# ViliamVadocz/tak

Measured on AMD Instinct MI355X. Metric: MCTS node-expansions/sec (5x5 Tak, 400 sims/move, 4096 games/GPU), higher is better.
Workload: dtype f32

## Files before the change

### tak_amd/csrc/conv_mainloop.cuh

```cuda
#pragma once
#include <hip/hip_runtime.h>
#include <stdint.h>

#include <utility>

namespace tg {

using f32x16 = __attribute__((ext_vector_type(16))) float;
using f32x4 = __attribute__((ext_vector_type(4))) float;
constexpr int LDS_PAD = 4;
constexpr int LDS_PAD16 = 8;


template <int RTW>
__device__ __forceinline__ void conv_tap_masks(int rows, int n, int nsq, int rho0, int (&vmask)[RTW]) {
#pragma unroll
    for (int j = 0; j < RTW; j++) {
        int rho = rho0 + j * 16;
        int p = rho / nsq;
        int sq = rho - p * nsq;
        int y = sq / n, x = sq - y * n;
        int m = 0;
#pragma unroll
        for (int t = 0; t < 9; t++) {
// ... 138 lines not shown
#pragma unroll
                for (int j = 0; j < H1; j++) { TG_HALO_MFMA(j, t, s) }
            __builtin_amdgcn_sched_barrier(0);
            if (SPLIT && s % CH == 0 && s > 0) {
#pragma unroll
                for (int j = H1; j < RTW; j++) { acc[j] += part[j]; asm volatile("" : "+v"(acc[j])); }
            }
            f32x4 w2;
            if (s < ROW - 2) {
                w2 = TG_HALO_W(wchunk);
            } else {
                const bool on = dy == 2;
                const __amdgpu_buffer_rsrc_t r = __builtin_amdgcn_make_buffer_rsrc((void*)(on ? wnext : wlayer), 0, (int)(9 * CH * WCHUNK), 0x00020000);
                w2 = __builtin_bit_cast(f32x4, __builtin_amdgcn_raw_buffer_load_b128(r, wlane, (int)((on ? s - (ROW - 2) : wchunk) * WCHUNK), 0));
            }
            wchunk++;
            if (s + 1 < ROW) {
#pragma unroll
                for (int j = 0; j < H1; j++) a[j] = lds4[ad[j] + TG_HALO_OFF2(s + 1)];
            } else {
#pragma unroll
                for (int j = H1; j < RTW; j++) ad[j] += RS * P4;
                if (dy < 2) {
#pragma unroll
                    for (int j = 0; j < H1; j++) { ad[j] += RS * P4; a[j] = lds4[ad[j] + TG_HALO_OFF2(0)]; }
                }
            }
            __builtin_amdgcn_sched_barrier(0);
#pragma unroll
            for (int t = 0; t < 4; t++)
#pragma unroll
                for (int j = H1; j < RTW; j++) { TG_HALO_MFMA(j, t, s) }
            __builtin_amdgcn_sched_barrier(0);
            if (SPLIT && s % CH == CH - 1) {
#pragma unroll
                for (int j = 0; j < (s == ROW - 1 ? RTW : H1); j++) { acc[j] += part[j]; asm volatile("" : "+v"(acc[j])); }
            }
            w0 = w1;
            w1 = w2;
        }
    }
#undef TG_HALO_MFMA
#undef TG_HALO_OFF2
#ifndef TG_NO_PRIO_TURNS
    __builtin_amdgcn_s_setprio(0);
#endif
#undef TG_HALO_OFF
#undef TG_HALO_W
}

constexpr int SQ_NB = 5;
template <int CH> constexpr int sq_image_cell4() { return 4 * CH + 2; }
template <int CH> constexpr int sq_image_pitch4() {
    constexpr int c = SQ_NB * SQ_NB * sq_image_cell4<CH>();
    return c + ((2 - c) % 16 + 16) % 16;
}
static_assert(sq_image_pitch4<4>() == 450, "C2: 16 positions = 115 200 B");
__host__ __device__ constexpr int sq_tiles(int rg) { return rg == 0 ? 13 : 12; }
__host__ __device__ constexpr int sq_tile(int rg, int j) { return rg == 0 ? (j < 12 ? j : 14) : (j < 2 ? 12 + j : 13 + j); }
__host__ __device__ constexpr bool sq_tap_on(int sq, int tap) {
    const int y = sq / SQ_NB + tap / 3 - 1, x = sq % SQ_NB + tap % 3 - 1;
    return y >= 0 && y < SQ_NB && x >= 0 && x < SQ_NB;
}
__host__ __device__ constexpr int sq_tap_count(int rg, int tap) {
    int c = 0;
    for (int j = 0; j < sq_tiles(rg); j++) c += sq_tap_on(sq_tile(rg, j), tap) ? 1 : 0;
    return c;
}
__host__ __device__ constexpr int sq_tap_tile(int rg, int tap, int k) {
    for (int j = 0; j < sq_tiles(rg); j++)
        if (sq_tap_on(sq_tile(rg, j), tap) && k-- == 0) return j;
    return -1;
}
static_assert(sq_tap_count(0, 0) + sq_tap_count(0, 1) + sq_tap_count(0, 2) + sq_tap_count(0, 3) + sq_tap_count(0, 4) + sq_tap_count(0, 5) +
                      sq_tap_count(0, 6) + sq_tap_count(0, 7) + sq_tap_count(0, 8) == 86, "row group 0: 86 on-board taps");
static_assert(sq_tap_count(1, 0) + sq_tap_count(1, 1) + sq_tap_count(1, 2) + sq_tap_count(1, 3) + sq_tap_count(1, 4) + sq_tap_count(1, 5) +
                      sq_tap_count(1, 6) + sq_tap_count(1, 7) + sq_tap_count(1, 8) == 83, "row group 1: 83 on-board taps");

template <typename Fn, int... I>
__device__ __forceinline__ void static_for_impl(Fn& f, std::integer_sequence<int, I...>) { (f(std::integral_constant<int, I>{}), ...); }
template <int N, typename Fn>
__device__ __forceinline__ void static_for(Fn&& f) { static_for_impl(f, std::make_integer_sequence<int, N>{}); }

template <int RG, int CH>
__device__ __forceinline__ void conv_mainloop_sq(const f32x4* __restrict__ img4, const float* __restrict__ wlayer,
                                                 const float* __restrict__ wnext, uint32_t wlane, f32x4 (&acc)[13], const int turn,
                                                 f32x4& w0, f32x4& w1) {
    constexpr int STEPS = 9 * CH, ROW = 3 * CH, CP4 = sq_image_cell4<CH>();
    constexpr size_t WCHUNK = (size_t)16 * CH * 4 * 16;
    static_assert(sq_tiles(RG) <= 13, "acc holds 13 tiles");
#ifndef TG_PRIO_PERIOD
#define TG_PRIO_PERIOD 2
#endif
    const __amdgpu_buffer_rsrc_t wrsrc = __builtin_amdgcn_make_buffer_rsrc((void*)wlayer, 0, (int)(9 * CH * WCHUNK), 0x00020000);
    const __amdgpu_buffer_rsrc_t nrsrc = __builtin_amdgcn_make_buffer_rsrc((void*)wnext, 0, (int)(9 * CH * WCHUNK), 0x00020000);
    constexpr auto cnt = [](int s) { return sq_tap_count(RG, s / CH); };
    constexpr auto h1 = [](int s) { return (sq_tap_count(RG, s / CH) + 1) / 2; };
    constexpr auto off = [](int s, int k) {
        return (sq_tile(RG, sq_tap_tile(RG, s / CH, k)) + (s / CH / 3 - 1) * SQ_NB + (s / CH % 3 - 1)) * CP4 + (s % CH) * 4;
    };
    f32x4 a1[7], a2[7];
    static_for<7>([&](auto K) {
        constexpr int k = decltype(K)::value;
        if constexpr (k < h1(0)) a1[k] = img4[off(0, k)];
    });
    static_for<STEPS>([&](auto S) {
        constexpr int s = decltype(S)::value;
#ifndef TG_NO_PRIO_TURNS
        if constexpr (s % TG_PRIO_PERIOD == 0) {
            if ((((s % ROW) / TG_PRIO_PERIOD + s / ROW) & 1) == turn) __builtin_amdgcn_s_setprio(1);
            else __builtin_amdgcn_s_setprio(0);
        }
#endif
        static_for<7>([&](auto K) {
            constexpr int k = decltype(K)::value;
            if constexpr (h1(s) + k < cnt(s)) a2[k] = img4[off(s, h1(s) + k)];
        });
        __builtin_amdgcn_sched_barrier(0);
        static_for<4>([&](auto T) {
            static_for<7>([&](auto K) {
                constexpr int t = decltype(T)::value, k = decltype(K)::value;
                if constexpr (k < h1(s)) {
                    constexpr int j = sq_tap_tile(RG, s / CH, k);
                    acc[j] = __builtin_amdgcn_mfma_f32_16x16x4f32(w0[t], a1[k][t], acc[j], 0, 0, 0);
                }
            });
        });
        __builtin_amdgcn_sched_barrier(0);
        f32x4 w2;
        if constexpr (s < STEPS - 2) w2 = __builtin_bit_cast(f32x4, __builtin_amdgcn_raw_buffer_load_b128(wrsrc, wlane, (int)((s + 2) * WCHUNK), 0));
        else w2 = __builtin_bit_cast(f32x4, __builtin_amdgcn_raw_buffer_load_b128(nrsrc, wlane, (int)((s - (STEPS - 2)) * WCHUNK), 0));
        if constexpr (s + 1 < STEPS) {
            static_for<7>([&](auto K) {
                constexpr int k = decltype(K)::value;
                if constexpr (k < h1(s + 1)) a1[k] = img4[off(s + 1, k)];
            });
        }
        __builtin_amdgcn_sched_barrier(0);
        static_for<4>([&](auto T) {
            static_for<7>([&](auto K) {
                constexpr int t = decltype(T)::value, k = decltype(K)::value;
                if constexpr (h1(s) + k < cnt(s)) {
                    constexpr int j = sq_tap_tile(RG, s / CH, h1(s) + k);
                    acc[j] = __builtin_amdgcn_mfma_f32_16x16x4f32(w0[t], a2[k][t], acc[j], 0, 0, 0);
                }
            });
        });
        __builtin_amdgcn_sched_barrier(0);
        w0 = w1;
        w1 = w2;
    });
#ifndef TG_NO_PRIO_TURNS
    __builtin_amdgcn_s_setprio(0);
#endif
}

template <int CH, int COT = CH>
__device__ __forceinline__ void conv_halo_first_weights(const float* __restrict__ wlayer, uint32_t wlane, f32x4& w0, f32x4& w1) {
    constexpr size_t WCHUNK = (size_t)16 * COT * 4 * 16;
    const __amdgpu_buffer_rsrc_t wrsrc = __builtin_amdgcn_make_buffer_rsrc((void*)wlayer, 0, (int)(9 * CH * WCHUNK), 0x00020000);
    w0 = __builtin_bit_cast(f32x4, __builtin_amdgcn_raw_buffer_load_b128(wrsrc, wlane, 0, 0));
    w1 = __builtin_bit_cast(f32x4, __builtin_amdgcn_raw_buffer_load_b128(wrsrc, wlane, (int)WCHUNK, 0));
}

}
```

### tak_amd/csrc/net.hip

```cpp
#include <cmath>
#include <cstdlib>
#include <cstring>

#include "engine.h"
#include "kernels.h"
#include "softmax.cuh"
#include "rng.cuh"

namespace tg {

struct ConvLayer {
    DevBuf w, b;
    int cin_pad = 0;
    int cout = 0, cout_pad = 0;
};

struct Net {
    std::map<std::string, std::vector<float>> tensors;
    bool ready = false;
    int F = 0, R = 0, cin = 0, cin_pad = 0;
    ConvLayer conv0;
    std::vector<ConvLayer> res1, res2;
    ConvLayer policy_conv;
    DevBuf policy_w, policy_b;
// ... 460 lines not shown
    TG_HIP(n->y.ensure(mb * nsq * F * 4));
    size_t logit_row = e->cfg.policy_head == TG_HEAD_CONV ? (size_t)nsq * n->policy_conv.cout_pad : (size_t)std::max(n->policy_np, n->s3_np);
    TG_HIP(n->logits.ensure(mb * logit_row * 4));
    TG_HIP(n->planes_nhwc.ensure(mb * nsq * n->cin_pad * 4));
    const bool s3fc = n->s3 && n->s3_fc_on;
    n->fc_stats_on = e->cfg.policy_head == TG_HEAD_FC5 && n->value_in_fc && !env_on("TG_NO_FC_STATS") && e->policy_size + 1 <= FC_TILES * 16 &&
                     (s3fc ? n->s3_np >= FC_TILES * 16 : fc_stats_supported(nsq * F, n->policy_np, n->policy_np));
    n->fc_stat_blocks = n->fc_stats_on ? FC_STAT_BLOCKS : 0;
    n->fc_stat_stride = n->fc_stats_on ? FC_STAT_STRIDE : 0;
    if (n->fc_stats_on) TG_HIP(n->fc_stats.ensure(mb * (size_t)n->fc_stat_stride * 2 * 4));
    n->ready = true;
    return TG_OK;
}

static int net_forward_impl(TgEngine* e, int nb, const float* d_planes, const uint8_t* d_states, float* d_policy, float* d_eval);

int net_forward_dev(TgEngine* e, int nb, const float* d_planes, float* d_policy, float* d_eval) {
    return net_forward_impl(e, nb, d_planes, nullptr, d_policy, d_eval);
}

bool net_takes_states(const TgEngine* e) { return net_ready(e) && (e->net->fused || e->net->s3); }

const float* net_fc_logits(const TgEngine* e, int* ld) {
    if (!net_ready(e)) return nullptr;
    const Net* n = e->net;
    if (e->cfg.policy_head != TG_HEAD_FC5 || !n->value_in_fc || e->policy_size > 2048) return nullptr;
    if (n->s3 && !n->s3_fc_on) return nullptr;
    *ld = n->s3 && n->s3_fc_on ? n->s3_np : n->policy_np;
    return n->logits.as<float>();
}

const float* net_fc_stats(const TgEngine* e, int* blocks, int* stride) {
    if (!net_ready(e) || !e->net->fc_stats_on) return nullptr;
    if (e->net->s3 && !e->net->s3_fc_on) return nullptr;
    *blocks = e->net->fc_stat_blocks;
    *stride = e->net->fc_stat_stride;
    return e->net->fc_stats.as<float>();
}

bool net_gather_ok(const TgEngine* e, int leaves) {
    if (!net_ready(e)) return false;
    const Net* n = e->net;
    static const bool off = env_on("TG_NO_FC_GATHER");
    if (off || e->cfg.policy_head != TG_HEAD_FC5 || !n->fc_stats_on || !n->value_in_fc) return false;
    if (n->s3) return n->s3_fc_on && n->s3_fc_ring_on && !env_on("TG_S3_NO_FC_RING") && fc_s3_ring_supported(leaves, e->g.nsq * n->F, e->policy_size + 1);
    return fc_gather_supported(leaves, e->g.nsq * n->F, n->policy_np);
}
void net_set_gather(TgEngine* e, const FcGatherArgs* g) {
    if (!e || !e->net) return;
    e->net->gather_on = g != nullptr;
    if (g) e->net->gather = *g;
}

int net_forward_states_dev(TgEngine* e, int nb, const uint8_t* d_states, float* d_policy, float* d_eval) {
    if (!net_ready(e)) return fail(TG_ERR_STATE, "network weights not finalized (tg_net_finalize)");
    if (nb <= 0) return TG_OK;
    if (e->net->fused || e->net->s3) return net_forward_impl(e, nb, nullptr, d_states, d_policy, d_eval);
    launch_encode_nhwc(e->stream, d_states, nb, e->g.n, e->net->planes_nhwc.as<float>(), e->net->cin_pad);
    TG_HIP(hipGetLastError());
    return net_forward_impl(e, nb, e->net->planes_nhwc.as<float>(), nullptr, d_policy, d_eval);
}

static int net_forward_impl(TgEngine* e, int nb, const float* d_planes, const uint8_t* d_states, float* d_policy, float* d_eval) {
    if (!net_ready(e)) return fail(TG_ERR_STATE, "network weights not finalized (tg_net_finalize)");
    if (nb <= 0) return TG_OK;
    if (nb > e->cfg.max_batch) return fail(TG_ERR_INVALID_ARG, "batch larger than max_batch");
    Net* n = e->net;
    hipStream_t st = e->stream;
    const int F = n->F, nsq = e->g.nsq, N = e->g.n;
    const int M = nb * nsq;
    float* x = n->x.as<float>();
    float* y = n->y.as<float>();
    std::vector<hipEvent_t>* chain = nullptr;
    if (n->prof_every > 0 && (n->prof_counter++ % (uint64_t)n->prof_every) == 0) {
        if (n->ev_chains.size() >= 256) {
            TG_HIP(hipStreamSynchronize(st));
            prof_collect(n);
        }
        n->ev_chains.emplace_back();
        chain = &n->ev_chains.back();
        n->conv_rows = M;
        n->conv_flops = (n->fused || n->s3) ? 2ll * M * 9 * ((long long)n->cin * F + 2ll * n->R * F * F) : 2ll * M * 9 * F * F;
        if (n->fused && !n->s3) {
            const long long c0 = (d_states && n->tower.cb) ? 16 + 4 * n->tower.cb_last_t : n->cin;
            const long long taps = tower_square_tiles(N, F, nb) ? (long long)nb * 169 : 9ll * M;
            n->conv_flops_exec = 2ll * M * 9 * c0 * F + 2ll * taps * 2ll * n->R * F * F;
        } else n->conv_flops_exec = n->conv_flops;
        chain->push_back(prof_event(n, st));
    }
    if (n->s3) {
        if (chain) chain->push_back(prof_event(n, st));
        const bool split_out = n->s3_fc_on || n->s3_head_on;
        TowerS3Params T3 = n->tower_s3;
        if (n->s3_head_on) T3.head_out = n->logits.as<float>();
        if (d_states) TG_HIP(launch_tower_s3_states(st, d_states, T3, x, nb, N, split_out));
        else TG_HIP(launch_tower_s3(st, d_planes, T3, x, nb, N, split_out));
        if (chain) chain->push_back(prof_event(n, st));
    } else if (n->fused) {
        if (chain) chain->push_back(prof_event(n, st));
        if (d_states) TG_HIP(launch_tower_states(st, d_states, n->tower, x, nb, N, n->split_buf.as<float>()));
        else TG_HIP(launch_tower(st, d_planes, n->tower, x, nb, N));
        if (chain) chain->push_back(prof_event(n, st));
    } else {
        TG_HIP(launch_conv3x3(st, d_planes, n->conv0.w.as<float>(), n->conv0.b.as<float>(), nullptr, x, M, N, n->cin_pad,
                              n->conv0.cout_pad, F, F, true));
        if (chain) chain->push_back(prof_event(n, st));
        for (int i = 0; i < n->R; i++) {
            TG_HIP(launch_conv3x3(st, x, n->res1[i].w.as<float>(), n->res1[i].b.as<float>(), nullptr, y, M, N, F,
                                  n->res1[i].cout_pad, F, F, true));
            if (chain) chain->push_back(prof_event(n, st));
            TG_HIP(launch_conv3x3(st, y, n->res2[i].w.as<float>(), n->res2[i].b.as<float>(), x, x, M, N, F,
                                  n->res2[i].cout_pad, F, F, true));
            if (chain) chain->push_back(prof_event(n, st));
        }
    }
    float* logits = n->logits.as<float>();
    bool value_done = false;
    if (e->cfg.policy_head == TG_HEAD_CONV) {
        const ConvLayer& L = n->policy_conv;
        if (!(n->s3 && n->s3_head_on))
            TG_HIP(launch_conv3x3(st, x, L.w.as<float>(), L.b.as<float>(), nullptr, logits, M, N, F, L.cout_pad, L.cout_pad, L.cout, false));
        const ValueHeadArgs vh{x, n->value_w.as<float>(), n->value_b, nsq * F, d_eval};
        const bool plain_value = !(n->s3 && (n->s3_fc_on || n->s3_head_on));
        TG_HIP(launch_softmax(st, logits, nsq * L.cout_pad, true, nsq, L.cout_pad, e->policy_size, nb, d_policy, nullptr, plain_value ? &vh : nullptr, &value_done));
    } else if (n->s3 && n->s3_fc_on) {
        float* stats = n->fc_stats_on ? n->fc_stats.as<float>() : nullptr;
        const bool gather = !d_policy && n->gather_on && net_gather_ok(e, nb);
        TG_HIP(launch_fc_s3(st, x, n->s3_fc.p, n->s3_fc_ring_on ? n->s3_fc_ring.p : nullptr, n->s3_fc_b.as<float>(), logits, nb, nsq * F, n->s3_np, n->s3_np,
                            e->policy_size + (n->value_in_fc ? 1 : 0), stats, e->policy_size, gather ? &n->gather : nullptr));
        if (d_policy && stats) TG_HIP(launch_softmax_stats(st, logits, n->s3_np, stats, n->fc_stat_blocks, n->fc_stat_stride, e->policy_size, nb, d_policy, d_eval));
        else if (d_policy) TG_HIP(launch_softmax(st, logits, n->s3_np, false, nsq, 0, e->policy_size, nb, d_policy, n->value_in_fc ? d_eval : nullptr));
    } else {
        float* stats = n->fc_stats_on ? n->fc_stats.as<float>() : nullptr;
        const bool gather = !d_policy && n->gather_on && net_gather_ok(e, nb);
        static const bool lin_src = !env_on("TG_FC_PERMUTED_SRC");
        TG_HIP(launch_gemm(st, x, nsq * F, n->policy_w.as<float>(), n->policy_b.as<float>(), logits, nb, nsq * F, n->policy_np,
                           n->policy_np, e->policy_size + (n->value_in_fc ? 1 : 0), !n->s3 && n->fused && n->tower.frag_out,
                           stats, e->policy_size, gather ? &n->gather : nullptr, lin_src ? n->policy_w_lin.as<float>() : nullptr));
        if (d_policy && stats) TG_HIP(launch_softmax_stats(st, logits, n->policy_np, stats, n->fc_stat_blocks, n->fc_stat_stride, e->policy_size, nb, d_policy, d_eval));
        else if (d_policy) TG_HIP(launch_softmax(st, logits, n->policy_np, false, nsq, 0, e->policy_size, nb, d_policy, n->value_in_fc ? d_eval : nullptr));
    }
    if (!d_policy && !(e->cfg.policy_head == TG_HEAD_FC5 && n->value_in_fc)) return fail(TG_ERR_STATE, "logits-only forward needs the FC head with the value column");
    if (e->cfg.policy_head == TG_HEAD_FC5 && n->value_in_fc) {
    } else if (n->s3 && (n->s3_fc_on || n->s3_head_on)) TG_HIP(launch_value_head_s3(st, x, n->value_w.as<float>(), n->value_b, nb, nsq * F, d_eval));
    else if (!value_done) TG_HIP(launch_value_head(st, x, n->value_w.as<float>(), n->value_b, nb, nsq * F, d_eval));
    if (chain) chain->push_back(prof_event(n, st));
    return TG_OK;
}

int net_poll_errors(TgEngine* e) {
    if (!e || !e->net || !e->net->split_ctl.p) return TG_OK;
    int err = 0;
    TG_HIP(hipMemcpy(&err, e->net->split_ctl.as<int>() + TOWER_SPLIT_CTL_WORDS - 32, 4, hipMemcpyDeviceToHost));
    if (!err) return TG_OK;
    TG_HIP(hipMemset(e->net->split_ctl.p, 0, (size_t)TOWER_SPLIT_CTL_WORDS * 4));
    return fail(TG_ERR_HIP, err == 2 ? "k_tower_split: the workgroups of one position ran on different XCDs (the same-L2 exchange is not safe on this "
                                       "device: set TG_SPLIT_AGENT_FENCES=1 or TG_NO_SPLIT_TOWER=1); the forward's results are invalid"
                                     : "k_tower_split: a workgroup waited for its position's siblings beyond the bound; the forward's results are invalid");
}

int net_profile_enable(TgEngine* e, int sample_every) {
    if (!e || !e->net) return fail(TG_ERR_STATE, "engine has no network (evaluator is not TG_EVAL_RESNET)");
    if (sample_every < 0) return fail(TG_ERR_INVALID_ARG, "sample_every must be >= 0");
    e->net->prof_every = sample_every;
    e->net->prof_counter = 0;
    return TG_OK;
}

int net_profile_read(TgEngine* e, TgProfile* out) {
// ... 145 lines not shown
```

### tak_amd/csrc/net_kernels.hip

```cpp
#include <hip/hip_runtime.h>
#include <stdint.h>
#include <stdlib.h>

#include <mutex>
#include <vector>

#include "board.cuh"
#include "conv_mainloop.cuh"
#include "fc_ring.cuh"
#include "softmax.cuh"
#include "tower_cb.cuh"
#include "kernels.h"

namespace tg {

#ifdef TG_TOWER_STAMPS
__device__ unsigned long long* g_tower_stamps = nullptr;
#define TG_STAMP(layer, slot)                                                                                       \
    do {                                                                                                            \
        if (blockIdx.x == 0 && g_tower_stamps && (threadIdx.x & 63) == 0)                                           \
            g_tower_stamps[((size_t)(layer) * 16 + (threadIdx.x >> 6)) * 8 + (slot)] = __builtin_amdgcn_s_memtime(); \
    } while (0)
#else
#define TG_STAMP(layer, slot) do { } while (0)
// ... 180 lines not shown

    f32x4 w_cur = wp[0];
    int kk = 0;
    for (int tap = 0; tap < 9; tap++) {
        const int dy = tap / 3 - 1, dx = tap % 3 - 1;
        int aoff[RTW];
#pragma unroll
        for (int j = 0; j < RTW; j++) {
            int yy = (pyx[j] & 0xff) + dy, xx = (pyx[j] >> 8) + dx;
            bool ok = yy >= 0 && yy < n && xx >= 0 && xx < n;
            aoff[j] = ok ? base4[j] + (dy * n + dx) * LS4 : zero4;
        }
        f32x4 a_cur[RTW];
#pragma unroll
        for (int j = 0; j < RTW; j++) a_cur[j] = lds4[aoff[j]];
        f32x4 part[RTW];
#pragma unroll
        for (int j = 0; j < RTW; j++) part[j] = f32x4{0.0f, 0.0f, 0.0f, 0.0f};
        for (int kc = 0; kc < chunks; kc++) {
            const int kkn = kk + 1 < total_chunks ? kk + 1 : kk;
            const f32x4 w_nxt = wp[(size_t)kkn * wstride4];
            const int kn = kc + 1 < chunks ? kc + 1 : kc;
            f32x4 a_nxt[RTW];
#pragma unroll
            for (int j = 0; j < RTW; j++) a_nxt[j] = lds4[aoff[j] + kn * 4];
#pragma unroll
            for (int t = 0; t < 4; t++)
#pragma unroll
                for (int j = 0; j < RTW; j++) part[j] = __builtin_amdgcn_mfma_f32_16x16x4f32(w_cur[t], a_cur[j][t], part[j], 0, 0, 0);
#pragma unroll
            for (int j = 0; j < RTW; j++) a_cur[j] = a_nxt[j];
            w_cur = w_nxt;
            kk++;
        }
#pragma unroll
        for (int j = 0; j < RTW; j++) acc[j] += part[j];
    }

    const int ch = ch0 + 4 * q;
    const f32x4 bv = *(const f32x4*)&bias[ch];
#pragma unroll
    for (int j = 0; j < RTW; j++) {
        int rho = (rg * RTW + j) * 16 + r16;
        if (rho < rows && ch < cout_valid) {
            size_t o = ((size_t)pos0 * nsq + rho) * out_stride + ch;
            f32x4 v = acc[j] + bv;
            if (res) v += *(const f32x4*)&res[o];
            if (relu) { v[0] = fmaxf(v[0], 0.0f); v[1] = fmaxf(v[1], 0.0f); v[2] = fmaxf(v[2], 0.0f); v[3] = fmaxf(v[3], 0.0f); }
            if (ch + 3 < cout_valid) *(f32x4*)&out[o] = v;
            else for (int t = 0; t < 4; t++) if (ch + t < cout_valid) out[o + t] = v[t];
        }
    }
}


template <int NWAVES>
__device__ __forceinline__ void tower_stage_states_cb(f32x4* lds4, f32x4* pb4, const uint8_t* states, int pos0, int npos, int n,
                                                      int LS4, const TowerParams& T) {
    const int wave = threadIdx.x >> 6, lane = threadIdx.x & 63;
    const Geom geo = make_geom(n);
    const int nsq = n * n;
    auto stage_one = [&](int p, const WRaw& raw) {
        WState ws;
        ws_unpack(ws, raw, geo);
        const float fcd = fcd_value(ws, geo);
        const RowMask m = ws_row_mask(ws, geo);
        if (lane < nsq) {
            f32x4* row = lds4 + (size_t)(p * nsq + lane) * LS4;
            f32x4 qd[8];
            tower_cb_board_quads(m, n, qd);
#pragma unroll
            for (int k = 0; k < 4; k++) row[k] = qd[k];
            const f32x4 lc[4] = {qd[4], qd[5], qd[6], qd[7]};
            conv_last_chunk_store(row + 4, lc, T.cb_last_t);
        }
        tower_cb_table(ws, fcd, n, p, T.F >> 2, (const f32x4*)T.cplane_sums, (const f32x4*)T.b[0], pb4);
    };
    for (int p = wave; p < npos; p += 2 * NWAVES) {
        const int p1 = p + NWAVES;
        const WRaw r0 = ws_load_raw(states + (size_t)(pos0 + p) * geo.bytes, geo);
        const WRaw r1 = ws_load_raw(states + (size_t)(pos0 + (p1 < npos ? p1 : p)) * geo.bytes, geo);
        stage_one(p, r0);
        if (p1 < npos) stage_one(p1, r1);
    }
}

template <int RTW, int NWAVES, int CH0, int CH, bool FROM_STATES, bool CB = false>
__global__ __launch_bounds__(NWAVES * 64) void k_tower(const float* __restrict__ in, TowerParams T, float* __restrict__ out,
                                                       int B, int n, int PW, int CTW) {
    static_assert(!CB || FROM_STATES, "the constant-plane bias needs the packed states");
    extern __shared__ __attribute__((aligned(16))) float lds[];
    f32x4* lds4 = (f32x4*)lds;
    const int tid = threadIdx.x;
    const int nsq = n * n;
    const int pos0 = blockIdx.x * PW;
    const int npos = min(PW, B - pos0);
    const int rows = npos * nsq;
    const int F = T.F;
    const int wave = tid >> 6, lane = tid & 63;
    const int ct = wave % CTW, rg = wave / CTW;
    const int r16 = lane & 15, q = lane >> 4;
    const int ch0 = ct * 16;

    int Cpad = CB ? T.cb_cin_pad : T.cin_pad;
    int LS4 = (Cpad + LDS_PAD16) >> 2;
    f32x4* pb4 = lds4 + (size_t)(PW * nsq + 1) * LS4;
    if (CB) {
        tower_stage_states_cb<NWAVES>(lds4, pb4, (const uint8_t*)in, pos0, npos, n, LS4, T);
        for (int idx = tid; idx < LS4; idx += NWAVES * 64) lds4[rows * LS4 + idx] = f32x4{0.0f, 0.0f, 0.0f, 0.0f};
    } else if (FROM_STATES) {
        const Geom geo = make_geom(n);
        const uint8_t* states = (const uint8_t*)in;
        const int C = input_channels(n);
        for (int p = wave; p < npos; p += NWAVES) {
            WState ws;
            ws_load(ws, states + (size_t)(pos0 + p) * geo.bytes, geo);
            const float fcd = fcd_value(ws, geo);
            const RowMask m = ws_row_mask(ws, geo);
            if (lane < nsq) {
                f32x4* row = lds4 + (size_t)(p * nsq + lane) * LS4;
                const int kl = (Cpad >> 2) - 4;
                for (int k = 0; k < kl; k++) {
                    float4 v = row_mask_value(m, k, C, fcd);
                    row[k] = f32x4{v.x, v.y, v.z, v.w};
                }
                f32x4 lc[4];
#pragma unroll
                for (int k = 0; k < 4; k++) {
                    float4 v = row_mask_value(m, kl + k, C, fcd);
                    lc[k] = f32x4{v.x, v.y, v.z, v.w};
                }
                conv_last_chunk_store(row + kl, lc, T.cin_last_t);
            }
        }
        for (int idx = tid; idx < LS4; idx += NWAVES * 64) lds4[rows * LS4 + idx] = f32x4{0.0f, 0.0f, 0.0f, 0.0f};
    } else {
        const int vpr = Cpad >> 2;
        const f32x4* src = (const f32x4*)(in + (size_t)pos0 * nsq * Cpad);
        const int total = rows * vpr;
        for (int idx = tid; idx < total; idx += NWAVES * 64) {
            int r = idx / vpr, v = idx - r * vpr;
            if (v < vpr - 4) lds4[r * LS4 + v] = src[idx];
        }
        for (int r = tid; r < rows; r += NWAVES * 64) {
            f32x4 lc[4];
#pragma unroll
            for (int k = 0; k < 4; k++) lc[k] = src[(size_t)r * vpr + vpr - 4 + k];
            conv_last_chunk_store(lds4 + (size_t)r * LS4 + vpr - 4, lc, T.cin_last_t);
        }
        for (int idx = tid; idx < LS4; idx += NWAVES * 64) lds4[rows * LS4 + idx] = f32x4{0.0f, 0.0f, 0.0f, 0.0f};
    }
    __syncthreads();

    const int NRG = NWAVES / CTW;
    const int ntiles = (PW * nsq + 15) >> 4;
    const int tbase = ntiles / NRG, trem = ntiles - tbase * NRG;
    const int my_tiles = tbase + (rg < trem ? 1 : 0);
    const int rho0 = (rg * tbase + min(rg, trem)) * 16 + r16;
    const bool short_group = my_tiles < RTW;

    f32x4 acc[RTW];
#pragma unroll
    for (int j = 0; j < RTW; j++) acc[j] = f32x4{0.0f, 0.0f, 0.0f, 0.0f};
    int vmask[RTW];
    conv_tap_masks<RTW>(rows, n, nsq, rho0, vmask);
    if (short_group) vmask[RTW - 1] = 0;
// ... 359 lines not shown
        __syncthreads();
        TG_STAMP(0, 5);
    }

    int cell4[RTW], rowid[RTW], addr4[RTW];
#pragma unroll
    for (int j = 0; j < RTW; j++) {
        const uint32_t e = j < my_tiles ? T.slotmap[(tile0 + j) * 16 + r16] : 0xFFFF0000u;
        rowid[j] = (int)(e >> 16);
        const bool idle = rowid[j] == 0xFFFF;
        cell4[j] = (idle ? LEAD + PW * PS : (int)(e & 0xFFFFu)) * P4 + (ch0 >> 2) + q;
        addr4[j] = ((idle ? LEAD + n * RS : (int)(e & 0xFFFFu)) - LEAD) * P4 + q;
    }
    const int turn = (wave >> 2) & 1;
    for (int layer = 1; layer < T.nlayers; layer++) {
#pragma unroll
        for (int j = 0; j < RTW; j++) asm volatile("" : "+v"(addr4[j]));
        TG_STAMP(layer, 0);
        const float* wnext = T.w[layer + 1 < T.nlayers ? layer + 1 : layer];
        const f32x4 bv = *(const f32x4*)&T.b[layer][ch0 + 4 * q];
        if (RTW > 1 && short_group) {
            f32x4 (&acs)[RTW - 1] = *reinterpret_cast<f32x4 (*)[RTW - 1]>(&acc[0]);
            conv_mainloop_halo<RTW - 1, CH, NB>(lds4, T.w[layer], wnext, wlane, addr4, acs, turn, w0, w1);
        } else {
            conv_mainloop_halo<RTW, CH, NB>(lds4, T.w[layer], wnext, wlane, addr4, acc, turn, w0, w1);
        }
        TG_STAMP(layer, 1);
#pragma unroll
        for (int j = 0; j < RTW; j++) {
            f32x4 v = acc[j] + bv;
            v[0] = fmaxf(v[0], 0.0f); v[1] = fmaxf(v[1], 0.0f); v[2] = fmaxf(v[2], 0.0f); v[3] = fmaxf(v[3], 0.0f);
            acc[j] = v;
        }
        if (layer + 1 == T.nlayers) {
#pragma unroll
            for (int j = 0; j < RTW; j++)
                if (rowid[j] < rows) {
                    if (T.frag_out) {
                        const int p = pos0 + rowid[j] / nsq, sq = rowid[j] % nsq;
                        ((f32x4*)out)[((size_t)(p >> 4) * (nsq * CH) + sq * CH + ct) * 64 + (p & 15) * 4 + q] = acc[j];
                    } else *(f32x4*)&out[((size_t)pos0 * nsq + rowid[j]) * F + ch0 + 4 * q] = acc[j];
                }
            break;
        }
        TG_STAMP(layer, 2);
        __syncthreads();
        TG_STAMP(layer, 3);
        const bool conv1 = (layer & 1) == 1;
#pragma unroll
        for (int j = 0; j < RTW; j++) {
            f32x4 x0 = f32x4{0.0f, 0.0f, 0.0f, 0.0f};
            if (conv1) x0 = lds4[cell4[j]];
            lds4[cell4[j]] = acc[j];
            acc[j] = x0;
        }
        TG_STAMP(layer, 4);
        __syncthreads();
        TG_STAMP(layer, 5);
    }
}

template <int RG, int CH>
__device__ __forceinline__ void tower_sq_store(const f32x4 (&acc)[13], const TowerParams& T, float* __restrict__ out, int p, int q, int ct) {
    constexpr int nsq = SQ_NB * SQ_NB;
#pragma unroll
    for (int j = 0; j < sq_tiles(RG); j++) {
        const int sq = sq_tile(RG, j);
        if (T.frag_out) ((f32x4*)out)[((size_t)(p >> 4) * (nsq * CH) + sq * CH + ct) * 64 + (p & 15) * 4 + q] = acc[j];
        else *(f32x4*)&out[((size_t)p * nsq + sq) * (16 * CH) + ct * 16 + 4 * q] = acc[j];
    }
}
template <int RG, int CH>
__device__ __forceinline__ void tower_sq_writeback(f32x4* cell4, f32x4 (&acc)[13], bool conv1) {
#pragma unroll
    for (int j = 0; j < sq_tiles(RG); j++) {
        const int o = sq_tile(RG, j) * sq_image_cell4<CH>();
        f32x4 x0 = f32x4{0.0f, 0.0f, 0.0f, 0.0f};
        if (conv1) x0 = cell4[o];
        cell4[o] = acc[j];
        acc[j] = x0;
    }
}

template <int CH0, bool FROM_STATES, bool CB = false>
__global__ __launch_bounds__(512) void k_tower_sq(const float* __restrict__ in, TowerParams T, float* __restrict__ out, int B) {
    static_assert(!CB || FROM_STATES, "the constant-plane bias needs the packed states");
    constexpr int RTW = 13, NWAVES = 8, CTW = 4, CH = 4, NB = SQ_NB, nsq = NB * NB, PW = 16;
    constexpr int PP4 = sq_image_pitch4<CH>(), CP4 = sq_image_cell4<CH>();
    extern __shared__ __attribute__((aligned(16))) float lds[];
    f32x4* lds4 = (f32x4*)lds;
    TG_STAMP(0, 6);
    const int tid = threadIdx.x;
    const int pos0 = blockIdx.x * PW;
    const int npos = min(PW, B - pos0);
    const int wave = tid >> 6, lane = tid & 63;
    const int ct = wave % CTW, rg = wave / CTW;
    const int r16 = lane & 15, q = lane >> 4;
    const int ch0 = ct * 16;
    const uint32_t wlane = (uint32_t)(((ch0 + r16) * 4 + q) * 16);
    f32x4 w0 = f32x4{0.0f, 0.0f, 0.0f, 0.0f}, w1 = w0;
    f32x4 acc[RTW];
    int rho0, my_tiles;
    tower_plain_layer0<RTW, NWAVES, CH0, CH, NB, FROM_STATES, CB>(in, T, lds4, PW, pos0, npos, CTW, wlane, acc, rho0, my_tiles, w0, w1);
    if (T.nlayers == 1) {
#pragma unroll
        for (int j = 0; j < RTW; j++) {
            const int rho = rho0 + j * 16;
            if (j < my_tiles && rho < npos * nsq) {
                const int p = pos0 + rho / nsq, sq = rho % nsq;
                if (T.frag_out) ((f32x4*)out)[((size_t)(p >> 4) * (nsq * CH) + sq * CH + ct) * 64 + (p & 15) * 4 + q] = acc[j];
                else *(f32x4*)&out[((size_t)pos0 * nsq + rho) * (16 * CH) + ch0 + 4 * q] = acc[j];
            }
        }
        return;
    }
    TG_STAMP(0, 2);
    __syncthreads();
    TG_STAMP(0, 3);
#pragma unroll
    for (int j = 0; j < RTW; j++) {
        const int rho = rho0 + j * 16;
        if (j < my_tiles) {
            const int p = rho / nsq, sq = rho - p * nsq;
            lds4[p * PP4 + sq * CP4 + (ch0 >> 2) + q] = acc[j];
        }
        acc[j] = f32x4{0.0f, 0.0f, 0.0f, 0.0f};
    }
    TG_STAMP(0, 4);
    __syncthreads();
    TG_STAMP(0, 5);

    int ad = r16 * PP4 + q;
    const int turn = rg;
    for (int layer = 1; layer < T.nlayers; layer++) {
        asm volatile("" : "+v"(ad));
        const f32x4* img4 = lds4 + ad;
        TG_STAMP(layer, 0);
        const float* wnext = T.w[layer + 1 < T.nlayers ? layer + 1 : layer];
        const f32x4 bv = *(const f32x4*)&T.b[layer][ch0 + 4 * q];
        if (rg == 0) conv_mainloop_sq<0, CH>(img4, T.w[layer], wnext, wlane, acc, turn, w0, w1);
        else conv_mainloop_sq<1, CH>(img4, T.w[layer], wnext, wlane, acc, turn, w0, w1);
        TG_STAMP(layer, 1);
#pragma unroll
        for (int j = 0; j < RTW; j++) {
            f32x4 v = acc[j] + bv;
            v[0] = fmaxf(v[0], 0.0f); v[1] = fmaxf(v[1], 0.0f); v[2] = fmaxf(v[2], 0.0f); v[3] = fmaxf(v[3], 0.0f);
            acc[j] = v;
        }
        if (layer + 1 == T.nlayers) {
            if (r16 < npos) {
                int p = pos0 + r16;
                asm volatile("" : "+v"(p));
                if (rg == 0) tower_sq_store<0, CH>(acc, T, out, p, q, ct);
                else tower_sq_store<1, CH>(acc, T, out, p, q, ct);
            }
            break;
        }
        TG_STAMP(layer, 2);
        __syncthreads();
        TG_STAMP(layer, 3);
        const bool conv1 = (layer & 1) == 1;
        f32x4* cell4 = lds4 + ad + (ch0 >> 2);
        if (rg == 0) tower_sq_writeback<0, CH>(cell4, acc, conv1);
        else tower_sq_writeback<1, CH>(cell4, acc, conv1);
        TG_STAMP(layer, 4);
        __syncthreads();
        TG_STAMP(layer, 5);
    }
}

template <int RTW, int NWAVES, int CH, int NB, int COT, int PSC>
__global__ __launch_bounds__(NWAVES * 64) void k_conv_halo(const float* __restrict__ in, const float* __restrict__ Wp,
                                                           const float* __restrict__ bias, const float* __restrict__ res,
                                                           float* __restrict__ out, const uint32_t* __restrict__ slotmap, int B, int PW,
                                                           int PS, int CTW, int out_stride, int cout_valid, int relu,
                                                           double* __restrict__ stats_part, const ConvBnBwdIn bnb) {
    extern __shared__ __attribute__((aligned(16))) float lds[];
    f32x4* lds4 = (f32x4*)lds;
    constexpr int n = NB, nsq = NB * NB, RS = NB + 1, LEAD = NB + 2, F4 = 4 * CH, P4 = 4 * CH + 1;
    PS = PSC;
    const int tid = threadIdx.x;
    const int pos0 = blockIdx.x * PW;
    const int npos = min(PW, B - pos0);
    const int rows = npos * nsq;
    const int wave = tid >> 6, lane = tid & 63;
    const int ct = wave % CTW, rg = wave / CTW;
    const int r16 = lane & 15, q = lane >> 4;
    const int ch0 = (blockIdx.y * CTW + ct) * 16;
    const uint32_t wlane = (uint32_t)(((ch0 + r16) * 4 + q) * 16);
    f32x4 w0, w1;
    TG_STAMP(0, 0);
#ifdef TG_TOWER_STAMPS
    if (g_tower_stamps && tid == 0) g_tower_stamps[128 + 2 * blockIdx.x] = __builtin_amdgcn_s_memrealtime();
#endif
    conv_halo_first_weights<CH, COT>(Wp, wlane, w0, w1);
    const int cells = LEAD + PW * PS + 1;
    for (int idx = tid; idx < cells * P4; idx += NWAVES * 64) {
        const int c = idx / P4 - LEAD;
        const int o = c < 0 || c >= PW * PS ? n * RS : c % PS;
        if (o >= n * RS || o % RS == n) lds4[idx] = f32x4{0.0f, 0.0f, 0.0f, 0.0f};
    }
    auto halo_cell = [&](int idx) {
        const int r = idx / F4, v = idx - r * F4;
        const int p = r / nsq, sq = r - p * nsq, y = sq / n, x = sq - y * n;
        return (LEAD + p * PS + y * RS + x) * P4 + v;
    };
    const f32x4* src = (const f32x4*)(in + (size_t)pos0 * nsq * (16 * CH));
    const int total = rows * F4;
    {
        constexpr int UNR = 8;
        for (int base = 0; base < total; base += NWAVES * 64 * UNR) {
            f32x4 tmp[UNR];
#pragma unroll
            for (int u = 0; u < UNR; u++) {
                const int idx = base + u * NWAVES * 64 + tid;
                tmp[u] = src[idx < total ? idx : total - 1];
// ... 794 lines not shown
    if (conv_lds_bytes(2, n, Cpad) > 160 * 1024) {
        if (CoutP % 128 == 0) return launch_conv_t<1, 2>(st, in, Wp, bias, res, out, M, n, Cpad, CoutP, out_stride, cout_valid, relu);
        return launch_conv_t<1, 1>(st, in, Wp, bias, res, out, M, n, Cpad, CoutP, out_stride, cout_valid, relu);
    }
    if (CoutP % 128 == 0) return launch_conv_t<2, 2>(st, in, Wp, bias, res, out, M, n, Cpad, CoutP, out_stride, cout_valid, relu);
    return launch_conv_t<2, 1>(st, in, Wp, bias, res, out, M, n, Cpad, CoutP, out_stride, cout_valid, relu);
}


static size_t tower_cb_table_bytes(int PW, int F) { return (size_t)PW * 9 * F * sizeof(float); }

template <int RTW, int NWAVES, int CH0, int CH, bool FROM_STATES, bool CB = false>
static hipError_t launch_tower_t(hipStream_t st, const float* in, const TowerParams& T, float* out, int B, int n, int PW, int CTW) {
    const size_t rows1 = (size_t)(PW * n * n + 1);
    const size_t first = rows1 * ((CB ? T.cb_cin_pad : T.cin_pad) + LDS_PAD16) * sizeof(float) + (CB ? tower_cb_table_bytes(PW, T.F) : 0);
    const size_t later = rows1 * (T.F + LDS_PAD16) * sizeof(float);
    const size_t lds = first > later ? first : later;
    static LdsAttr lds_attr;
    if (hipError_t e = lds_attr.ensure((const void*)k_tower<RTW, NWAVES, CH0, CH, FROM_STATES, CB>, lds); e != hipSuccess) return e;
    hipLaunchKernelGGL((k_tower<RTW, NWAVES, CH0, CH, FROM_STATES, CB>), dim3((B + PW - 1) / PW), dim3(NWAVES * 64), lds, st, in, T, out, B, n, PW, CTW);
    return hipGetLastError();
}


bool tower_halo_geometry(int n, int F, int* pw, int* ps) {
    if (n == 5 && F == 64) { *pw = 16; *ps = 36; return true; }
    if (n == 5 && F == 128) { *pw = 8; *ps = 37; return true; }
    if (n == 6 && F == 128) { *pw = 4; *ps = 51; return true; }
    return false;
}

void tower_halo_slotmap(int n, int pw, int ps, uint32_t* out) {
    const int nsq = n * n, RS = n + 1, LEAD = n + 2, rows = pw * nsq, tiles = (rows + 15) / 16;
    std::vector<std::vector<int>> bucket(16);
    std::vector<int> cell(rows);
    for (int r = rows - 1; r >= 0; r--) {
        const int p = r / nsq, sq = r % nsq;
        cell[r] = LEAD + p * ps + (sq / n) * RS + sq % n;
        bucket[cell[r] % 16].push_back(r);
    }
    static const int outer[8] = {0, 1, 2, 3, 12, 13, 14, 15}, inner[8] = {4, 5, 6, 7, 8, 9, 10, 11};
    for (int t = 0; t < tiles; t++) {
        size_t left[2] = {0, 0};
        for (int r = 0; r < 16; r++) left[r & 1] += bucket[r].size();
        const int par = left[0] >= left[1] ? 0 : 1;
        for (const int* slots : {outer, inner}) {
            int missing[8], nm = 0;
            for (int k = 0; k < 8; k++) {
                std::vector<int>& b = bucket[2 * k + par];
                if (!b.empty()) { out[t * 16 + slots[k]] = (uint32_t)cell[b.back()] | ((uint32_t)b.back() << 16); b.pop_back(); }
                else missing[nm++] = slots[k];
            }
            for (int m = 0; m < nm; m++) {
                int big = 0;
                for (int r = 1; r < 16; r++) if (bucket[r].size() > bucket[big].size()) big = r;
                if (!bucket[big].empty()) {
                    out[t * 16 + missing[m]] = (uint32_t)cell[bucket[big].back()] | ((uint32_t)bucket[big].back() << 16);
                    bucket[big].pop_back();
                } else out[t * 16 + missing[m]] = 0xFFFF0000u;
            }
        }
    }
}

template <int RTW, int NWAVES, int CH0, int CH, int NB, bool FROM_STATES, bool CB = false>
static hipError_t launch_tower_halo_t(hipStream_t st, const float* in, const TowerParams& T, float* out, int B, int CTW) {
    const int PW = T.halo_pw;
    const size_t plain = (size_t)(PW * NB * NB + 1) * ((CB ? T.cb_cin_pad : T.cin_pad) + LDS_PAD16) * sizeof(float) +
                         (CB ? tower_cb_table_bytes(PW, 16 * CH) : 0);
    const size_t halo = (size_t)(NB + 2 + PW * T.halo_ps + 1) * (16 * CH + 4) * sizeof(float);
    const size_t lds = plain > halo ? plain : halo;
    static LdsAttr lds_attr;
    if (hipError_t e = lds_attr.ensure((const void*)k_tower_halo<RTW, NWAVES, CH0, CH, NB, FROM_STATES, CB>, lds); e != hipSuccess) return e;
    hipLaunchKernelGGL((k_tower_halo<RTW, NWAVES, CH0, CH, NB, FROM_STATES, CB>), dim3((B + PW - 1) / PW), dim3(NWAVES * 64), lds, st, in, T, out, B, PW, CTW);
    return hipGetLastError();
}

template <int CH0, bool FROM_STATES, bool CB = false>
static hipError_t launch_tower_sq_t(hipStream_t st, const float* in, const TowerParams& T, float* out, int B) {
    constexpr int PW = 16, NB = SQ_NB, CH = 4;
    const size_t plain = (size_t)(PW * NB * NB + 1) * ((CB ? T.cb_cin_pad : T.cin_pad) + LDS_PAD16) * sizeof(float) +
                         (CB ? tower_cb_table_bytes(PW, 16 * CH) : 0);
    const size_t image = (size_t)PW * sq_image_pitch4<CH>() * 16;
    const size_t lds = plain > image ? plain : image;
    static LdsAttr lds_attr;
    if (hipError_t e = lds_attr.ensure((const void*)k_tower_sq<CH0, FROM_STATES, CB>, lds); e != hipSuccess) return e;
    hipLaunchKernelGGL((k_tower_sq<CH0, FROM_STATES, CB>), dim3((B + PW - 1) / PW), dim3(512), lds, st, in, T, out, B);
    return hipGetLastError();
}

bool tower_square_tiles(int n, int F, int B) {
    static const bool off = env_on("TG_NO_HALO_TOWER");
    return !off && n == SQ_NB && F == 64 && B > 2048;
}

template <bool FROM_STATES>
static bool launch_tower_halo(hipStream_t st, const float* in, const TowerParams& T, float* out, int B, int n, hipError_t* err) {
    static const bool off = env_on("TG_NO_HALO_TOWER");
    if (off || !T.slotmap) return false;
    if (FROM_STATES && T.cb) {
        if (tower_square_tiles(n, T.F, B)) { *err = launch_tower_sq_t<2, FROM_STATES, FROM_STATES>(st, in, T, out, B); return true; }
        if (n == 6 && T.F == 128 && B > 512) { *err = launch_tower_halo_t<9, 8, 2, 8, 6, FROM_STATES, FROM_STATES>(st, in, T, out, B, 8); return true; }
        if (n == 5 && T.F == 128 && B > 1024) { *err = launch_tower_halo_t<13, 8, 2, 8, 5, FROM_STATES, FROM_STATES>(st, in, T, out, B, 8); return true; }
        return false;
    }
    if (tower_square_tiles(n, T.F, B) && T.cin_pad == 80) { *err = launch_tower_sq_t<5, FROM_STATES>(st, in, T, out, B); return true; }
    if (n == 6 && T.F == 128 && T.cin_pad == 96 && B > 512) { *err = launch_tower_halo_t<9, 8, 6, 8, 6, FROM_STATES>(st, in, T, out, B, 8); return true; }
    if (n == 5 && T.F == 128 && T.cin_pad == 80 && B > 1024) { *err = launch_tower_halo_t<13, 8, 5, 8, 5, FROM_STATES>(st, in, T, out, B, 8); return true; }
    return false;
}

bool tower_supported(int n, int F, int cin_pad) {
    if (n == 5 && F == 64 && cin_pad == 80) return true;
    if (n == 6 && F == 128 && cin_pad == 96) return true;
    if (n == 5 && F == 128 && cin_pad == 80) return true;
    return false;
}

__global__ void k_xcc_probe(unsigned* __restrict__ out) {
    unsigned x;
    asm volatile("s_getreg_b32 %0, hwreg(HW_REG_XCC_ID)" : "=s"(x));
    if (threadIdx.x == 0) out[blockIdx.x] = x & 15u;
}
static bool workgroups_round_robin_over_xcds() {
    static std::mutex guard;
    static int verdict[16] = {};
    std::lock_guard<std::mutex> lock(guard);
    int dev = 0;
    if (hipGetDevice(&dev) != hipSuccess || dev < 0 || dev >= 16) return false;
    if (verdict[dev]) return verdict[dev] == 1;
    verdict[dev] = 2;
    unsigned* d = nullptr;
    unsigned h[64];
    if (hipMalloc((void**)&d, sizeof(h)) != hipSuccess) return false;
    bool ok = true;
    for (int rep = 0; rep < 4 && ok; rep++) {
        hipLaunchKernelGGL(k_xcc_probe, dim3(64), dim3(64), 0, nullptr, d);
        ok = hipMemcpy(h, d, sizeof(h), hipMemcpyDeviceToHost) == hipSuccess;
        for (int i = 8; i < 64 && ok; i++) ok = h[i] == h[i & 7];
    }
    (void)hipFree(d);
    if (ok) verdict[dev] = 1;
    return ok;
}

template <int NRT, int CTW, int CH>
static hipError_t launch_tower_split_t(hipStream_t st, const uint8_t* states, const TowerParams& T, float* out, float* scratch, int B, int n) {
    const int nsq = n * n, F = 16 * CH;
    const size_t first = (size_t)(nsq + 1) * (T.cb_cin_pad + LDS_PAD16) * sizeof(float) + tower_cb_table_bytes(1, F);
    const size_t later = (size_t)(nsq + 1) * (F + LDS_PAD16) * sizeof(float);
    const size_t lds = first > later ? first : later;
    constexpr int G = CH / CTW;
    const dim3 grid((B + 7) / 8 * 8 * G), block(NRT * CTW * 64);
    static const bool agent_fences = env_on("TG_SPLIT_AGENT_FENCES");
    if (!agent_fences && workgroups_round_robin_over_xcds()) {
        static LdsAttr lds_attr;
        if (hipError_t e = lds_attr.ensure((const void*)k_tower_split<NRT, CTW, CH, true>, lds); e != hipSuccess) return e;
        hipLaunchKernelGGL((k_tower_split<NRT, CTW, CH, true>), grid, block, lds, st, states, T, out, scratch, B, n);
    } else {
        static LdsAttr lds_attr;
        if (hipError_t e = lds_attr.ensure((const void*)k_tower_split<NRT, CTW, CH, false>, lds); e != hipSuccess) return e;
        hipLaunchKernelGGL((k_tower_split<NRT, CTW, CH, false>), grid, block, lds, st, states, T, out, scratch, B, n);
    }
    return hipGetLastError();
}

static bool launch_tower_split(hipStream_t st, const uint8_t* states, const TowerParams& T, float* out, float* scratch, int B, int n,
// ... 116 lines not shown
```

Measured before the change: 5.879 million.

## Run constant-plane layer 0 through the square-tile conv mainloop

For the fused-from-states constant-plane path, layer 0 now stages the board planes directly into the square-tile LDS image and runs the same square-tile MFMA mainloop used by the residual layers. The mainloop gains a reduced input-channel count and a partial-last-chunk mask, so only on-board taps are computed and trailing zero channels are skipped. The previous generic plain layer-0 routine, with its extra LDS round-trip and separate tiling, is bypassed. This adds a per-class bias epilogue and requires cb_cin_pad==32 and cb_last_t==3, otherwise the launch returns an error.

```diff
diff --git a/tak_amd/csrc/conv_mainloop.cuh b/tak_amd/csrc/conv_mainloop.cuh
--- a/tak_amd/csrc/conv_mainloop.cuh
+++ b/tak_amd/csrc/conv_mainloop.cuh
@@ -244,22 +244,22 @@
 template <int N, typename Fn>
 __device__ __forceinline__ void static_for(Fn&& f) { static_for_impl(f, std::make_integer_sequence<int, N>{}); }
 
-template <int RG, int CH>
+template <int RG, int CH, int CHL = CH, int LAST_T = 4>
 __device__ __forceinline__ void conv_mainloop_sq(const f32x4* __restrict__ img4, const float* __restrict__ wlayer,
                                                  const float* __restrict__ wnext, uint32_t wlane, f32x4 (&acc)[13], const int turn,
                                                  f32x4& w0, f32x4& w1) {
-    constexpr int STEPS = 9 * CH, ROW = 3 * CH, CP4 = sq_image_cell4<CH>();
+    constexpr int STEPS = 9 * CHL, ROW = 3 * CHL, CP4 = sq_image_cell4<CH>();
     constexpr size_t WCHUNK = (size_t)16 * CH * 4 * 16;
     static_assert(sq_tiles(RG) <= 13, "acc holds 13 tiles");
 #ifndef TG_PRIO_PERIOD
 #define TG_PRIO_PERIOD 2
 #endif
-    const __amdgpu_buffer_rsrc_t wrsrc = __builtin_amdgcn_make_buffer_rsrc((void*)wlayer, 0, (int)(9 * CH * WCHUNK), 0x00020000);
+    const __amdgpu_buffer_rsrc_t wrsrc = __builtin_amdgcn_make_buffer_rsrc((void*)wlayer, 0, (int)(STEPS * WCHUNK), 0x00020000);
     const __amdgpu_buffer_rsrc_t nrsrc = __builtin_amdgcn_make_buffer_rsrc((void*)wnext, 0, (int)(9 * CH * WCHUNK), 0x00020000);
-    constexpr auto cnt = [](int s) { return sq_tap_count(RG, s / CH); };
-    constexpr auto h1 = [](int s) { return (sq_tap_count(RG, s / CH) + 1) / 2; };
+    constexpr auto cnt = [](int s) { return sq_tap_count(RG, s / CHL); };
+    constexpr auto h1 = [](int s) { return (sq_tap_count(RG, s / CHL) + 1) / 2; };
     constexpr auto off = [](int s, int k) {
-        return (sq_tile(RG, sq_tap_tile(RG, s / CH, k)) + (s / CH / 3 - 1) * SQ_NB + (s / CH % 3 - 1)) * CP4 + (s % CH) * 4;
+        return (sq_tile(RG, sq_tap_tile(RG, s / CHL, k)) + (s / CHL / 3 - 1) * SQ_NB + (s / CHL % 3 - 1)) * CP4 + (s % CHL) * 4;
     };
     f32x4 a1[7], a2[7];
     static_for<7>([&](auto K) {
@@ -282,8 +282,8 @@
         static_for<4>([&](auto T) {
             static_for<7>([&](auto K) {
                 constexpr int t = decltype(T)::value, k = decltype(K)::value;
-                if constexpr (k < h1(s)) {
-                    constexpr int j = sq_tap_tile(RG, s / CH, k);
+                if constexpr (k < h1(s) && (s % CHL + 1 < CHL || t < LAST_T)) {
+                    constexpr int j = sq_tap_tile(RG, s / CHL, k);
                     acc[j] = __builtin_amdgcn_mfma_f32_16x16x4f32(w0[t], a1[k][t], acc[j], 0, 0, 0);
                 }
             });
@@ -302,8 +302,8 @@
         static_for<4>([&](auto T) {
             static_for<7>([&](auto K) {
                 constexpr int t = decltype(T)::value, k = decltype(K)::value;
-                if constexpr (h1(s) + k < cnt(s)) {
-                    constexpr int j = sq_tap_tile(RG, s / CH, h1(s) + k);
+                if constexpr (h1(s) + k < cnt(s) && (s % CHL + 1 < CHL || t < LAST_T)) {
+                    constexpr int j = sq_tap_tile(RG, s / CHL, h1(s) + k);
                     acc[j] = __builtin_amdgcn_mfma_f32_16x16x4f32(w0[t], a2[k][t], acc[j], 0, 0, 0);
                 }
             });
diff --git a/tak_amd/csrc/net.hip b/tak_amd/csrc/net.hip
--- a/tak_amd/csrc/net.hip
+++ b/tak_amd/csrc/net.hip
@@ -566,9 +566,10 @@
         n->conv_rows = M;
         n->conv_flops = (n->fused || n->s3) ? 2ll * M * 9 * ((long long)n->cin * F + 2ll * n->R * F * F) : 2ll * M * 9 * F * F;
         if (n->fused && !n->s3) {
-            const long long c0 = (d_states && n->tower.cb) ? 16 + 4 * n->tower.cb_last_t : n->cin;
+            const bool cb0 = d_states && n->tower.cb;
+            const long long c0 = cb0 ? 16 + 4 * n->tower.cb_last_t : n->cin;
             const long long taps = tower_square_tiles(N, F, nb) ? (long long)nb * 169 : 9ll * M;
-            n->conv_flops_exec = 2ll * M * 9 * c0 * F + 2ll * taps * 2ll * n->R * F * F;
+            n->conv_flops_exec = 2ll * (cb0 ? taps : 9ll * M) * c0 * F + 2ll * taps * 2ll * n->R * F * F;
         } else n->conv_flops_exec = n->conv_flops;
         chain->push_back(prof_event(n, st));
     }
diff --git a/tak_amd/csrc/net_kernels.hip b/tak_amd/csrc/net_kernels.hip
--- a/tak_amd/csrc/net_kernels.hip
+++ b/tak_amd/csrc/net_kernels.hip
@@ -286,6 +286,40 @@
         const WRaw r1 = ws_load_raw(states + (size_t)(pos0 + (p1 < npos ? p1 : p)) * geo.bytes, geo);
         stage_one(p, r0);
         if (p1 < npos) stage_one(p1, r1);
+    }
+}
+template <int NWAVES, int CH>
+__device__ __forceinline__ void tower_stage_states_cb_sq(f32x4* lds4, f32x4* pb4, const uint8_t* states, int pos0, int npos,
+                                                         const TowerParams& T) {
+    constexpr int n = SQ_NB, nsq = n * n, PW = 16, PP4 = sq_image_pitch4<CH>(), CP4 = sq_image_cell4<CH>(), LAST_T = 3;
+    const int wave = threadIdx.x >> 6, lane = threadIdx.x & 63;
+    const Geom geo = make_geom(n);
+    auto stage_one = [&](int p, const WRaw& raw) {
+        WState ws;
+        ws_unpack(ws, raw, geo);
+        const float fcd = fcd_value(ws, geo);
+        const RowMask m = ws_row_mask(ws, geo);
+        if (lane < nsq) {
+            f32x4* cell = lds4 + p * PP4 + lane * CP4;
+            f32x4 qd[8];
+            tower_cb_board_quads(m, n, qd);
+#pragma unroll
+            for (int k = 0; k < 4; k++) cell[k] = qd[k];
+            const f32x4 lc[4] = {qd[4], qd[5], qd[6], qd[7]};
+            conv_last_chunk_store(cell + 4, lc, LAST_T);
+        }
+        tower_cb_table(ws, fcd, n, p, 4 * CH, (const f32x4*)T.cplane_sums, (const f32x4*)T.b[0], pb4);
+    };
+    for (int p = wave; p < npos; p += 2 * NWAVES) {
+        const int p1 = p + NWAVES;
+        const WRaw r0 = ws_load_raw(states + (size_t)(pos0 + p) * geo.bytes, geo);
+        const WRaw r1 = ws_load_raw(states + (size_t)(pos0 + (p1 < npos ? p1 : p)) * geo.bytes, geo);
+        stage_one(p, r0);
+        if (p1 < npos) stage_one(p1, r1);
+    }
+    for (int idx = threadIdx.x; idx < (PW - npos) * nsq * 8; idx += NWAVES * 64) {
+        const int c = idx >> 3;
+        lds4[(npos + c / nsq) * PP4 + (c % nsq) * CP4 + (idx & 7)] = f32x4{0.0f, 0.0f, 0.0f, 0.0f};
     }
 }
 
@@ -811,6 +845,19 @@
     }
 }
 
+template <int RG, int CH>
+__device__ __forceinline__ void tower_sq_cb_epilogue(const f32x4* pbq, f32x4 (&acc)[13]) {
+#pragma unroll
+    for (int j = 0; j < sq_tiles(RG); j++) {
+        constexpr int n = SQ_NB;
+        const int sq = sq_tile(RG, j), y = sq / n, x = sq % n;
+        const int cls = (y == 0 ? 0 : y == n - 1 ? 2 : 1) * 3 + (x == 0 ? 0 : x == n - 1 ? 2 : 1);
+        f32x4 v = acc[j] + pbq[cls * 4 * CH];
+        v[0] = fmaxf(v[0], 0.0f); v[1] = fmaxf(v[1], 0.0f); v[2] = fmaxf(v[2], 0.0f); v[3] = fmaxf(v[3], 0.0f);
+        acc[j] = v;
+    }
+}
+
 template <int CH0, bool FROM_STATES, bool CB = false>
 __global__ __launch_bounds__(512) void k_tower_sq(const float* __restrict__ in, TowerParams T, float* __restrict__ out, int B) {
     static_assert(!CB || FROM_STATES, "the constant-plane bias needs the packed states");
@@ -829,38 +876,75 @@
     const uint32_t wlane = (uint32_t)(((ch0 + r16) * 4 + q) * 16);
     f32x4 w0 = f32x4{0.0f, 0.0f, 0.0f, 0.0f}, w1 = w0;
     f32x4 acc[RTW];
-    int rho0, my_tiles;
-    tower_plain_layer0<RTW, NWAVES, CH0, CH, NB, FROM_STATES, CB>(in, T, lds4, PW, pos0, npos, CTW, wlane, acc, rho0, my_tiles, w0, w1);
-    if (T.nlayers == 1) {
+    int ad = r16 * PP4 + q;
+    const int turn = rg;
+    if constexpr (CB) {
+        static_assert(CH0 == 2, "board planes: 32 channels");
+        f32x4* pb4 = lds4 + PW * PP4;
+        tower_stage_states_cb_sq<NWAVES, CH>(lds4, pb4, (const uint8_t*)in, pos0, npos, T);
+        conv_halo_first_weights<CH0, CH>(T.w0_board, wlane, w0, w1);
+        __syncthreads();
+#pragma unroll
+        for (int j = 0; j < RTW; j++) acc[j] = f32x4{0.0f, 0.0f, 0.0f, 0.0f};
+        asm volatile("" : "+v"(ad));
+        TG_STAMP(0, 0);
+        const float* wnext = T.nlayers > 1 ? T.w[1] : T.w0_board;
+        if (rg == 0) conv_mainloop_sq<0, CH, CH0, 3>(lds4 + ad, T.w0_board, wnext, wlane, acc, turn, w0, w1);
+        else conv_mainloop_sq<1, CH, CH0, 3>(lds4 + ad, T.w0_board, wnext, wlane, acc, turn, w0, w1);
+        TG_STAMP(0, 1);
+        const f32x4* pbq = pb4 + (r16 < npos ? r16 : 0) * 9 * 4 * CH + (ch0 >> 2) + q;
+        if (rg == 0) tower_sq_cb_epilogue<0, CH>(pbq, acc);
+        else tower_sq_cb_epilogue<1, CH>(pbq, acc);
+        if (T.nlayers == 1) {
+            if (r16 < npos) {
+                int p = pos0 + r16;
+                asm volatile("" : "+v"(p));
+                if (rg == 0) tower_sq_store<0, CH>(acc, T, out, p, q, ct);
+                else tower_sq_store<1, CH>(acc, T, out, p, q, ct);
+            }
+            return;
+        }
+        TG_STAMP(0, 2);
+        __syncthreads();
+        TG_STAMP(0, 3);
+        f32x4* cell4 = lds4 + ad + (ch0 >> 2);
+        if (rg == 0) tower_sq_writeback<0, CH>(cell4, acc, false);
+        else tower_sq_writeback<1, CH>(cell4, acc, false);
+        TG_STAMP(0, 4);
+        __syncthreads();
+        TG_STAMP(0, 5);
+    } else {
+        int rho0, my_tiles;
+        tower_plain_layer0<RTW, NWAVES, CH0, CH, NB, FROM_STATES, CB>(in, T, lds4, PW, pos0, npos, CTW, wlane, acc, rho0, my_tiles, w0, w1);
+        if (T.nlayers == 1) {
+#pragma unroll
+            for (int j = 0; j < RTW; j++) {
+                const int rho = rho0 + j * 16;
+                if (j < my_tiles && rho < npos * nsq) {
+                    const int p = pos0 + rho / nsq, sq = rho % nsq;
+                    if (T.frag_out) ((f32x4*)out)[((size_t)(p >> 4) * (nsq * CH) + sq * CH + ct) * 64 + (p & 15) * 4 + q] = acc[j];
+                    else *(f32x4*)&out[((size_t)pos0 * nsq + rho) * (16 * CH) + ch0 + 4 * q] = acc[j];
+                }
+            }
+            return;
+        }
+        TG_STAMP(0, 2);
+        __syncthreads();
+        TG_STAMP(0, 3);
 #pragma unroll
         for (int j = 0; j < RTW; j++) {
             const int rho = rho0 + j * 16;
-            if (j < my_tiles && rho < npos * nsq) {
-                const int p = pos0 + rho / nsq, sq = rho % nsq;
-                if (T.frag_out) ((f32x4*)out)[((size_t)(p >> 4) * (nsq * CH) + sq * CH + ct) * 64 + (p & 15) * 4 + q] = acc[j];
-                else *(f32x4*)&out[((size_t)pos0 * nsq + rho) * (16 * CH) + ch0 + 4 * q] = acc[j];
-            }
-        }
-        return;
-    }
-    TG_STAMP(0, 2);
-    __syncthreads();
-    TG_STAMP(0, 3);
-#pragma unroll
-    for (int j = 0; j < RTW; j++) {
-        const int rho = rho0 + j * 16;
-        if (j < my_tiles) {
-            const int p = rho / nsq, sq = rho - p * nsq;
-            lds4[p * PP4 + sq * CP4 + (ch0 >> 2) + q] = acc[j];
-        }
-        acc[j] = f32x4{0.0f, 0.0f, 0.0f, 0.0f};
-    }
-    TG_STAMP(0, 4);
-    __syncthreads();
-    TG_STAMP(0, 5);
-
-    int ad = r16 * PP4 + q;
-    const int turn = rg;
+            if (j < my_tiles) {
+                const int p = rho / nsq, sq = rho - p * nsq;
+                lds4[p * PP4 + sq * CP4 + (ch0 >> 2) + q] = acc[j];
+            }
+            acc[j] = f32x4{0.0f, 0.0f, 0.0f, 0.0f};
+        }
+        TG_STAMP(0, 4);
+        __syncthreads();
+        TG_STAMP(0, 5);
+    }
+
     for (int layer = 1; layer < T.nlayers; layer++) {
         asm volatile("" : "+v"(ad));
         const f32x4* img4 = lds4 + ad;
@@ -1821,7 +1905,8 @@
     const size_t plain = (size_t)(PW * NB * NB + 1) * ((CB ? T.cb_cin_pad : T.cin_pad) + LDS_PAD16) * sizeof(float) +
                          (CB ? tower_cb_table_bytes(PW, 16 * CH) : 0);
     const size_t image = (size_t)PW * sq_image_pitch4<CH>() * 16;
-    const size_t lds = plain > image ? plain : image;
+    if (CB && (T.cb_cin_pad != 32 || T.cb_last_t != 3)) return hipErrorInvalidValue;
+    const size_t lds = CB ? image + tower_cb_table_bytes(PW, 16 * CH) : plain > image ? plain : image;
     static LdsAttr lds_attr;
     if (hipError_t e = lds_attr.ensure((const void*)k_tower_sq<CH0, FROM_STATES, CB>, lds); e != hipSuccess) return e;
     hipLaunchKernelGGL((k_tower_sq<CH0, FROM_STATES, CB>), dim3((B + PW - 1) / PW), dim3(512), lds, st, in, T, out, B);
```

Measured after the change: 5.986 million (median of 6 runs). +1.8%, better.
